# 30stomercury/whisper-char-alignment

Measured on AMD Instinct MI355X. Metric: utterances/sec (whisper-medium, 10s audio, char align) at 1/2/4/8 MI355X, higher is better.
Workload: dtype f16x2 (hi + lo operand pairs on the f16 MFMA pipe: fp32-equivalent operands, fp32 accumulate)

## Files before the change

whisper-char-alignment_amd/csrc/gemm.hip:

```cpp
#include <atomic>

#include "gemm_epilogue.h"
#include <cstdlib>
#include "kernels.h"
#include "wca_common.h"

namespace wca {

namespace {

constexpr int BM = 128, BN = 128, BK = 64;
constexpr int TILE_ELEMS = 128 * 64;

struct RowPtrs {
  const half_t* p[4];
};

__device__ __forceinline__ half8 ldfrag(const half_t* tile, int r, int c) {
  return *reinterpret_cast<const half8*>(tile + r * 64 + ((c ^ swz128(r)) << 3));
}

template <int OUT_MODE, bool GELU, int MT>
__device__ __forceinline__ void epilogue(const GemmArgs& a, f32x4 (&acc)[MT][4], int mbase, int nb, int fr) {
  float bv[16];
#pragma unroll
  for (int j = 0; j < 16; ++j) bv[j] = (a.bias != nullptr && nb + j < a.N) ? a.bias[nb + j] : 0.f;
  const bool full_n = (nb + 16 <= a.N);

#pragma unroll
  for (int mt = 0; mt < MT; ++mt) {
    const int m = mbase + mt * 16 + fr;
    if (m >= a.M) continue;
    float v[16];
#pragma unroll
    for (int nt = 0; nt < 4; ++nt)
#pragma unroll
      for (int r = 0; r < 4; ++r) v[nt * 4 + r] = acc[mt][nt][r] + bv[nt * 4 + r];
    if (OUT_MODE != 2 && a.addend != nullptr) {
      const float* ap = a.addend + (long)m * a.ld_addend + nb;
#pragma unroll
      for (int j = 0; j < 16; ++j)
        if (nb + j < a.N) v[j] += ap[j];
    }
    if (GELU) {
#pragma unroll
      for (int j = 0; j < 16; j += 2) {
        if (OUT_MODE == 4) {
          const f32x2 g = gelu_erfc2(f32x2{v[j], v[j + 1]});
          v[j] = g[0];
          v[j + 1] = g[1];
        } else {
          v[j] = gelu_erf(v[j]);
          v[j + 1] = gelu_erf(v[j + 1]);
        }
      }
    }
    if (a.pos != nullptr) {
      const float* pp = a.pos + (long)(m % a.pos_period) * a.N + nb;
#pragma unroll
      for (int j = 0; j < 16; ++j)
        if (nb + j < a.N) v[j] += pp[j];
    }
    long coff;
    if (a.c_rows_per_batch > 0) {
      const int b = m / a.c_rows_per_batch;
      const int t = m - b * a.c_rows_per_batch;
      coff = (long)b * a.c_batch_stride + (long)t * a.ldc;
    } else {
      coff = (long)m * a.ldc;
    }
    if (OUT_MODE == 0 || OUT_MODE == 4) {
      half_t* cp = reinterpret_cast<half_t*>(a.C) + coff + nb;
      if (full_n && ((reinterpret_cast<uintptr_t>(cp) & 15) == 0)) {
        half8 h0, h1, l0, l1;
        if (OUT_MODE == 4) {
#pragma unroll
          for (int j = 0; j < 8; j += 2) {
            const Half2Pair p0 = split_pair2(v[j], v[j + 1]), p1 = split_pair2(v[8 + j], v[8 + j + 1]);
            h0[j] = p0.hi[0];
            h0[j + 1] = p0.hi[1];
            l0[j] = p0.lo[0];
            l0[j + 1] = p0.lo[1];
            h1[j] = p1.hi[0];
            h1[j + 1] = p1.hi[1];
            l1[j] = p1.lo[0];
            l1[j + 1] = p1.lo[1];
          }
        } else {
#pragma unroll
          for (int j = 0; j < 8; ++j) {
            h0[j] = (half_t)v[j];
            h1[j] = (half_t)v[8 + j];
          }
        }
        reinterpret_cast<half8*>(cp)[0] = h0;
        reinterpret_cast<half8*>(cp)[1] = h1;
        if (OUT_MODE == 4) {
          reinterpret_cast<half8*>(cp + a.c_lo)[0] = l0;
          reinterpret_cast<half8*>(cp + a.c_lo)[1] = l1;
        }
      } else {
#pragma unroll
        for (int j = 0; j < 16; ++j)
          if (nb + j < a.N) {
            if (OUT_MODE == 4) {
              const HalfPair pr = split_pair(v[j]);
              cp[j] = pr.hi;
              cp[a.c_lo + j] = pr.lo;
            } else {
              cp[j] = (half_t)v[j];
            }
          }
      }
    } else {
      float* cp = reinterpret_cast<float*>(a.C) + coff + nb;
      if (full_n && ((reinterpret_cast<uintptr_t>(cp) & 15) == 0)) {
        f32x4* c4 = reinterpret_cast<f32x4*>(cp);
#pragma unroll
        for (int q = 0; q < 4; ++q) {
          f32x4 o = f32x4{v[q * 4 + 0], v[q * 4 + 1], v[q * 4 + 2], v[q * 4 + 3]};
          if (OUT_MODE == 2) o += c4[q];
          c4[q] = o;
        }
      } else {
#pragma unroll
        for (int j = 0; j < 16; ++j)
          if (nb + j < a.N) cp[j] = (OUT_MODE == 2) ? cp[j] + v[j] : v[j];
      }
    }
  }
}

template <int OUT_MODE, bool GELU, int SITE>
__global__ __launch_bounds__(256, 2) void gemm_f16_kernel(GemmArgs a) {
  extern __shared__ __attribute__((aligned(16))) char smem[];
  half_t* lds = reinterpret_cast<half_t*>(smem);
  const int tid = threadIdx.x;
  const int lane = tid & 63;
  const int wave = __builtin_amdgcn_readfirstlane(tid >> 6);
  const int wm = wave >> 1, wn = wave & 1;

  const int ntn = (a.N + BN - 1) / BN;
  const int ntm = (a.M + BM - 1) / BM;
  const int nwg = ntm * ntn;
  const int id = xcd_remap(blockIdx.x, nwg);
  const int tm = id / ntn, tn = id - tm * ntn;
  const int m0 = tm * BM, n0 = tn * BN;

  const half_t* asrc[4];
  const half_t* wsrc[4];
#pragma unroll
  for (int i = 0; i < 4; ++i) {
    const int r = (wave * 4 + i) * 8 + (lane >> 3);
    const int c = (lane & 7) ^ swz128(r);
    int gm = m0 + r;
    gm = gm < a.M ? gm : a.M - 1;
    long aoff;
    if (a.a_rows_per_batch > 0) {
      const int b = gm / a.a_rows_per_batch;
      const int t = gm - b * a.a_rows_per_batch;
      aoff = (long)b * a.a_batch_stride + (long)t * a.lda;
    } else {
      aoff = (long)gm * a.lda;
    }
    const int kbeg = (int)blockIdx.y * (a.K / (int)gridDim.y);
    asrc[i] = a.A + aoff + c * 8 + kbeg;
    int gn = n0 + r;
    gn = gn < a.N ? gn : a.N - 1;
    wsrc[i] = a.W + (long)gn * a.ldw + c * 8 + kbeg;
  }

  auto stage = [&](int buf, int k0) {
    half_t* At = lds + buf * (2 * TILE_ELEMS);
    half_t* Wt = At + TILE_ELEMS;
#pragma unroll
    for (int i = 0; i < 4; ++i) {
      const int rbase = (wave * 4 + i) * 8;
      glds16(asrc[i] + k0, At + rbase * 64);
      glds16(wsrc[i] + k0, Wt + rbase * 64);
    }
  };

  f32x4 acc[4][4];
#pragma unroll
  for (int i = 0; i < 4; ++i)
#pragma unroll
    for (int j = 0; j < 4; ++j) acc[i][j] = f32x4{0.f, 0.f, 0.f, 0.f};

  const int fr = lane & 15;
  const int fg = lane >> 4;
  int xrow[4], wrow[4];
#pragma unroll
  for (int t = 0; t < 4; ++t) {
    xrow[t] = wm * 64 + t * 16 + fr;
    wrow[t] = wn * 64 + (fr >> 2) * 16 + t * 4 + (fr & 3);
  }

  const int nk = a.K / BK / (int)gridDim.y;
  stage(0, 0);
  wait_vm0();
  __syncthreads();
  int cur = 0;
  for (int kt = 0; kt < nk; ++kt) {
    if (kt + 1 < nk) stage(cur ^ 1, (kt + 1) * BK);
    const half_t* At = lds + cur * (2 * TILE_ELEMS);
    const half_t* Wt = At + TILE_ELEMS;
#pragma unroll
    for (int ks = 0; ks < 2; ++ks) {
      half8 xf[4], wf[4];
#pragma unroll
      for (int t = 0; t < 4; ++t) {
        xf[t] = ldfrag(At, xrow[t], ks * 4 + fg);
        wf[t] = ldfrag(Wt, wrow[t], ks * 4 + fg);
      }
#pragma unroll
      for (int mt = 0; mt < 4; ++mt)
#pragma unroll
        for (int nt = 0; nt < 4; ++nt)
          acc[mt][nt] = __builtin_amdgcn_mfma_f32_16x16x32_f16(wf[nt], xf[mt], acc[mt][nt], 0, 0, 0);
    }
    wait_vm0();
    __syncthreads();
    cur ^= 1;
  }

  if (OUT_MODE == 2 && gridDim.y > 1) {
    GemmArgs p = a;
    p.C = a.sk_part + (long)blockIdx.y * a.M * a.N;
    p.ldc = a.N;
    p.c_rows_per_batch = 0;
    p.bias = nullptr;
    p.pos = nullptr;
    epilogue<1, false, 4>(p, acc, m0 + wm * 64, n0 + wn * 64 + fg * 16, fr);
    return;
  }
  epilogue<OUT_MODE, GELU, 4>(a, acc, m0 + wm * 64, n0 + wn * 64 + fg * 16, fr);
}

__global__ __launch_bounds__(256) void splitk_reduce_kernel(const float* __restrict__ part, int S, int M, int N, const float* __restrict__ bias,
                                                            float* __restrict__ x, int ldc) {
  const long i4 = (long)blockIdx.x * blockDim.x + threadIdx.x;
  const int n4 = N >> 2;
  if (i4 >= (long)M * n4) return;
  const int m = (int)(i4 / n4), n = (int)(i4 - (long)m * n4) * 4;
  f32x4 v = *reinterpret_cast<const f32x4*>(part + (long)m * N + n);
  for (int s = 1; s < S; ++s) v += *reinterpret_cast<const f32x4*>(part + ((long)s * M + m) * N + n);
  if (bias != nullptr) v += *reinterpret_cast<const f32x4*>(bias + n);
  f32x4* xp = reinterpret_cast<f32x4*>(x + (long)m * ldc + n);
  *xp = *xp + v;
}


template <int OUT_MODE, bool GELU, int SITE>
__global__ __launch_bounds__(512) void gemm256_f16_kernel(GemmArgs a) {
  extern __shared__ __attribute__((aligned(16))) char smem[];
  half_t* lds = reinterpret_cast<half_t*>(smem);
  constexpr int TILE256 = 256 * 64;
  const int tid = threadIdx.x;
  const int lane = tid & 63;
  const int wave = __builtin_amdgcn_readfirstlane(tid >> 6);
  const int wr = wave >> 2, wc = wave & 3;

  const int ntn = (a.N + 255) / 256;
  const int ntm = (a.M + 255) / 256;
  const int nwg = ntm * ntn;
  const int id = xcd_remap(blockIdx.x, nwg);
  const int tm = id / ntn, tn = id - tm * ntn;
  const int m0 = tm * 256, n0 = tn * 256;

  const half_t* asrc[4];
  const half_t* wsrc[4];
#pragma unroll
  for (int i = 0; i < 4; ++i) {
    const int r = (wave * 4 + i) * 8 + (lane >> 3);
    const int c = (lane & 7) ^ swz128(r);
    int gm = m0 + r;
    gm = gm < a.M ? gm : a.M - 1;
    long aoff;
    if (a.a_rows_per_batch > 0) {
      const int b = gm / a.a_rows_per_batch;
      const int t = gm - b * a.a_rows_per_batch;
      aoff = (long)b * a.a_batch_stride + (long)t * a.lda;
    } else {
      aoff = (long)gm * a.lda;
    }
    asrc[i] = a.A + aoff + c * 8;
    int gn = n0 + r;
    gn = gn < a.N ? gn : a.N - 1;
    wsrc[i] = a.W + (long)gn * a.ldw + c * 8;
  }

  auto stage = [&](int buf, int k0) {
    half_t* At = lds + buf * (2 * TILE256);
    half_t* Wt = At + TILE256;
#pragma unroll
    for (int i = 0; i < 4; ++i) {
      const int rbase = (wave * 4 + i) * 8;
      glds16(asrc[i] + k0, At + rbase * 64);
      glds16(wsrc[i] + k0, Wt + rbase * 64);
    }
  };

  f32x4 acc[8][4];
#pragma unroll
  for (int i = 0; i < 8; ++i)
#pragma unroll
    for (int j = 0; j < 4; ++j) acc[i][j] = f32x4{0.f, 0.f, 0.f, 0.f};

  const int fr = lane & 15, fg = lane >> 4;
  int xrow[8], wrow[4];
#pragma unroll
  for (int t = 0; t < 8; ++t) xrow[t] = wr * 128 + t * 16 + fr;
#pragma unroll
  for (int t = 0; t < 4; ++t) wrow[t] = wc * 64 + (fr >> 2) * 16 + t * 4 + (fr & 3);

  const int nk = a.K / BK;
  stage(0, 0);
  if (nk > 1) stage(1, BK);
  for (int kt = 0; kt < nk; ++kt) {
    const int cur = kt & 1;
    const half_t* At = lds + cur * (2 * TILE256);
    const half_t* Wt = At + TILE256;
    if (kt + 1 < nk) {
      asm volatile("s_waitcnt vmcnt(8)" ::: "memory");
    } else {
      asm volatile("s_waitcnt vmcnt(0)" ::: "memory");
    }
    __builtin_amdgcn_s_barrier();
    asm volatile("" ::: "memory");

    half8 wf[2][4], xf[2][4];
#pragma unroll
    for (int ks = 0; ks < 2; ++ks)
#pragma unroll
      for (int t = 0; t < 4; ++t) {
        wf[ks][t] = ldfrag(Wt, wrow[t], ks * 4 + fg);
        xf[ks][t] = ldfrag(At, xrow[t], ks * 4 + fg);
      }
    __builtin_amdgcn_s_setprio(1);
#pragma unroll
    for (int ks = 0; ks < 2; ++ks)
#pragma unroll
      for (int mt = 0; mt < 4; ++mt)
#pragma unroll
        for (int nt = 0; nt < 4; ++nt)
          acc[mt][nt] = __builtin_amdgcn_mfma_f32_16x16x32_f16(wf[ks][nt], xf[ks][mt], acc[mt][nt], 0, 0, 0);
    __builtin_amdgcn_s_setprio(0);

    half8 xg[2][4];
#pragma unroll
    for (int ks = 0; ks < 2; ++ks)
#pragma unroll
      for (int t = 0; t < 4; ++t) xg[ks][t] = ldfrag(At, xrow[4 + t], ks * 4 + fg);
    asm volatile("s_waitcnt lgkmcnt(0)" ::: "memory");
    __builtin_amdgcn_s_barrier();
    asm volatile("" ::: "memory");
    if (kt + 2 < nk) stage(cur, (kt + 2) * BK);
    __builtin_amdgcn_s_setprio(1);
#pragma unroll
    for (int ks = 0; ks < 2; ++ks)
#pragma unroll
      for (int mt = 0; mt < 4; ++mt)
#pragma unroll
        for (int nt = 0; nt < 4; ++nt)
          acc[4 + mt][nt] = __builtin_amdgcn_mfma_f32_16x16x32_f16(wf[ks][nt], xg[ks][mt], acc[4 + mt][nt], 0, 0, 0);
    __builtin_amdgcn_s_setprio(0);
  }

  epilogue<OUT_MODE, GELU, 8>(a, acc, m0 + wr * 128, n0 + wc * 64 + fg * 16, fr);
}

template <int V>
struct GemmIntC {
  static constexpr int value = V;
};

template <int OUT_MODE, bool GELU, int SITE, int SPLITW_MODE = 0>
__global__ __launch_bounds__(512) void gemm256p_f16_kernel(GemmArgs a) {
  constexpr bool SPLITW = SPLITW_MODE != 0;
  constexpr bool RING3 = SPLITW_MODE == 2;
  extern __shared__ __attribute__((aligned(16))) char smem[];
  half_t* lds = reinterpret_cast<half_t*>(smem);
  constexpr int TILE256 = 256 * 64;
  float* bias_lds = reinterpret_cast<float*>(smem + 4 * TILE256 * sizeof(half_t));
  float* gamma_lds = bias_lds + 512;
  float* beta_lds = gamma_lds + 512;
  float* ln_lds = beta_lds + 512;
  const int tid = threadIdx.x;
  const int lane = tid & 63;
  const int wave = __builtin_amdgcn_readfirstlane(tid >> 6);
  const int wr = wave >> 2, wc = wave & 3;

  const int ntn = (a.N + 255) / 256;
  const int ntm = (a.M + 255) / 256;
  const int nwg = ntm * ntn;
  const int G = gridDim.x;

  const __amdgpu_buffer_rsrc_t ra = __builtin_amdgcn_make_buffer_rsrc(const_cast<half_t*>(a.A), 0, (int)a.a_bytes, 0x00020000);
  const __amdgpu_buffer_rsrc_t rw = __builtin_amdgcn_make_buffer_rsrc(const_cast<half_t*>(a.W), 0, (int)a.w_bytes, 0x00020000);
  const __amdgpu_buffer_rsrc_t rb = __builtin_amdgcn_make_buffer_rsrc(const_cast<float*>(a.bias), 0, a.bias != nullptr ? a.N * 4 : 0, 0x00020000);
  const __amdgpu_buffer_rsrc_t rg = __builtin_amdgcn_make_buffer_rsrc(const_cast<float*>(a.ln_gamma), 0, OUT_MODE == 3 ? a.N * 4 : 0, 0x00020000);
  const __amdgpu_buffer_rsrc_t rbeta = __builtin_amdgcn_make_buffer_rsrc(const_cast<float*>(a.ln_beta), 0, OUT_MODE == 3 ? a.N * 4 : 0, 0x00020000);
  const int l8 = lane >> 3;
  const int rho = wave * 8 + l8;
  const int c0 = (lane & 7) ^ ((rho >> 1) & 7);
  const int nt_r = rho >> 4, i_r = rho & 15;
  const int wsrc_row = (OUT_MODE == 0 || OUT_MODE == 3 || OUT_MODE == 4) ? ((nt_r >> 1) * 32 + (i_r >> 2) * 8 + (nt_r & 1) * 4 + (i_r & 3)) : rho;
  const unsigned va = (unsigned)(rho * a.lda + c0 * 8) * 2u;
  const unsigned vw = (unsigned)(wsrc_row * a.ldw + c0 * 8) * 2u;
  const unsigned sa64 = 64u * a.lda * 2u, sw64 = 64u * a.ldw * 2u;

  auto a_slot = [&](int buf) -> half_t* { return RING3 ? lds + buf * TILE256 : lds + buf * (2 * TILE256); };
  auto w_slot = [&](int bufw) -> half_t* { return RING3 ? lds + 3 * TILE256 : lds + bufw * (2 * TILE256) + TILE256; };
  auto stage_one = [&](int buf, int bufw, unsigned ta, unsigned tw, int g) {
    half_t* At = a_slot(buf);
    half_t* Wt = w_slot(bufw);
    const int i = g >> 1;
    unsigned so = ((g & 1) == 0) ? ta + i * sa64 : tw + i * sw64;
    asm volatile("" : "+s"(so));
    if ((g & 1) == 0)
      __builtin_amdgcn_raw_ptr_buffer_load_lds(ra, (WCA_LDS void*)(At + (i * 64 + wave * 8) * 64), 16, (int)(va + so), 0, 0, 0);
    else
      __builtin_amdgcn_raw_ptr_buffer_load_lds(rw, (WCA_LDS void*)(Wt + (i * 64 + wave * 8) * 64), 16, (int)(vw + so), 0, 0, 0);
  };

  auto stage_bias = [&](int par, int ncol0) {
    if (wave < 4) {
      __builtin_amdgcn_raw_ptr_buffer_load_lds(rb, (WCA_LDS void*)(bias_lds + par * 256 + wave * 64), 4, (ncol0 + wave * 64 + lane) * 4, 0, 0, 0);
      if (OUT_MODE == 3) {
        __builtin_amdgcn_raw_ptr_buffer_load_lds(rg, (WCA_LDS void*)(gamma_lds + par * 256 + wave * 64), 4, (ncol0 + wave * 64 + lane) * 4, 0, 0, 0);
        __builtin_amdgcn_raw_ptr_buffer_load_lds(rbeta, (WCA_LDS void*)(beta_lds + par * 256 + wave * 64), 4, (ncol0 + wave * 64 + lane) * 4, 0, 0, 0);
      }
    }
  };
  constexpr int RING3_A_REQS_IN_FLIGHT = 4;
  static_assert(RING3_A_REQS_IN_FLIGHT * 64 == 256, "one request per 64-row block of the 256-row A tile");

  const int fr = lane & 15, fg = lane >> 4;
  const int pos0 = fg ^ ((fr >> 1) & 7);
  const int xb0 = (wr * 128 + fr) * 64 + pos0 * 8, xb1 = (wr * 128 + fr) * 64 + (pos0 ^ 4) * 8;
  const int wb0 = (wc * 64 + fr) * 64 + pos0 * 8, wb1 = (wc * 64 + fr) * 64 + (pos0 ^ 4) * 8;

#define WCA_LOAD_HALF(AT, WT, XB, WB, WF, XF)                                                      \
  do {                                                                                             \
    _Pragma("unroll") for (int t = 0; t < 4; ++t) WF[t] = *reinterpret_cast<const half8*>((WT) + (WB) + t * 1024); \
    _Pragma("unroll") for (int t = 0; t < 8; ++t) XF[t] = *reinterpret_cast<const half8*>((AT) + (XB) + t * 1024); \
  } while (0)

  const int nk = SPLITW ? 2 * (a.K / BK) : a.K / BK;
  auto a_koff = [&](int s_) -> unsigned {
    return SPLITW ? (unsigned)(((s_ & 1) * (int)a.a_lo + (s_ >> 1) * BK) * 2) : (unsigned)(s_ * (BK * 2));
  };
  auto w_koff = [&](int s_) -> unsigned {
    return SPLITW ? (unsigned)((s_ >> 1) * (BK * 2)) : (unsigned)(s_ * (BK * 2));
  };
  int v = blockIdx.x;
  int id = xcd_remap(v, nwg);
  const int SM = a.supertile > 0 ? a.supertile : 1;
  auto tile_of = [&](int t, int& tm, int& tn) {
    const int per = SM * ntn;
    const int st = t / per, r = t - st * per;
    const int rows = (ntm - st * SM) < SM ? (ntm - st * SM) : SM;
    tn = r / rows;
    tm = st * SM + (r - tn * rows);
  };
  const int spx = G >> 3;
  const int PR = spx / ntn;
  const int lab = blockIdx.x & 7, slot = blockIdx.x >> 3;
  const int pq = ntm >> 3, prm = ntm & 7;
  const int lab_panels = pq + (lab < prm ? 1 : 0), lab_base = lab * pq + (lab < prm ? lab : prm);
  auto tile_of_round = [&](int round, int& tm, int& tn) -> bool {
    tn = slot / PR;
    const int pi = round * PR + (slot - tn * PR);
    tm = lab_base + pi;
    return tn < ntn && pi < lab_panels;
  };
  int tm_, tn_;
  int round = 0;
  if (OUT_MODE == 3) {
    if (!tile_of_round(0, tm_, tn_)) return;
  } else {
    tile_of(id, tm_, tn_);
  }
  int m0 = tm_ * 256, n0 = tn_ * 256;
  unsigned ta = (unsigned)m0 * a.lda * 2u, tw = (unsigned)n0 * a.ldw * 2u;

  f32x4 acc[8][4];
#pragma unroll
  for (int i = 0; i < 8; ++i)
#pragma unroll
    for (int j = 0; j < 4; ++j) acc[i][j] = f32x4{0.f, 0.f, 0.f, 0.f};
  half8 w0[4], x0[8], w1[4], x1[8];
  int par = 0;
  stage_bias(0, n0);
#pragma unroll
  for (int g = 0; g < 8; ++g) stage_one(0, 0, ta, tw, g);
  if (nk > 1) {
#pragma unroll
    for (int g = 0; g < 8; ++g)
      if (!SPLITW || (g & 1) == 0) stage_one(1, 1, ta + a_koff(1), tw + w_koff(1), g);
    if (SPLITW) asm volatile("s_waitcnt vmcnt(4)" ::: "memory");
    else asm volatile("s_waitcnt vmcnt(8)" ::: "memory");
  } else {
    asm volatile("s_waitcnt vmcnt(0)" ::: "memory");
  }
  __builtin_amdgcn_s_barrier();
  asm volatile("" ::: "memory");
  WCA_LOAD_HALF(a_slot(0), w_slot(0), xb0, wb0, w0, x0);
  int ring_a = 0;

  for (;;) {
    const int vn = v + G;
    bool has_next;
    int idn = id;
    int tmn_, tnn_;
    if (OUT_MODE == 3) {
      has_next = tile_of_round(round + 1, tmn_, tnn_);
      if (!has_next) {
        tmn_ = m0 >> 8;
        tnn_ = n0 >> 8;
      }
    } else {
      has_next = vn < nwg;
      idn = has_next ? xcd_remap(vn, nwg) : id;
      tile_of(idn, tmn_, tnn_);
    }
    const int m0n = tmn_ * 256, n0n = tnn_ * 256;
    const unsigned tan = (unsigned)m0n * a.lda * 2u, twn = (unsigned)n0n * a.ldw * 2u;
    auto kstep = [&](auto par_c, const int kt) {
      constexpr int PAR = decltype(par_c)::value;
      const int cur = RING3 ? ring_a : (PAR >= 0 ? PAR : (kt & 1));
      const int nxt = RING3 ? (ring_a == 2 ? 0 : ring_a + 1) : (cur ^ 1);
      const int wslot = SPLITW ? ((kt >> 1) & 1) : cur;
      const int wslot_n = SPLITW ? (((kt + 1) >> 1) & 1) : (cur ^ 1);
      const bool W_FRESH = !SPLITW || (PAR >= 0 ? PAR == 0 : (kt & 1) == 0);
      const bool W_NEXT_FRESH = !SPLITW || (PAR >= 0 ? PAR == 1 : (kt & 1) == 1);
      const half_t* At = a_slot(cur);
      const half_t* Wt = w_slot(wslot);
      const bool in_tile2 = kt + 2 < nk;
      const bool more1 = kt + 1 < nk, more2 = in_tile2 || has_next;
      const unsigned ka = (in_tile2 ? ta + a_koff(kt + 2) : tan + a_koff(kt + 2 - nk));
      const unsigned kw = (in_tile2 ? tw + w_koff(kt + 2) : twn + w_koff(kt + 2 - nk));
      const int prv = RING3 ? (ring_a == 0 ? 2 : ring_a - 1) : 0;
#pragma unroll
      for (int g = 0; g < 8; ++g) {
        __builtin_amdgcn_s_setprio(1);
#pragma unroll
        for (int nt = 0; nt < 4; ++nt) acc[g][nt] = __builtin_amdgcn_mfma_f32_16x16x32_f16(w0[nt], x0[g], acc[g][nt], 0, 0, 0);
        __builtin_amdgcn_s_setprio(0);
        __builtin_amdgcn_sched_barrier(0);
        if (g < 2) {
          if (W_FRESH) {
            w1[2 * g] = *reinterpret_cast<const half8*>(Wt + wb1 + (2 * g) * 1024);
            w1[2 * g + 1] = *reinterpret_cast<const half8*>(Wt + wb1 + (2 * g + 1) * 1024);
          }
        } else if (g < 6) {
          x1[2 * (g - 2)] = *reinterpret_cast<const half8*>(At + xb1 + (2 * (g - 2)) * 1024);
          x1[2 * (g - 2) + 1] = *reinterpret_cast<const half8*>(At + xb1 + (2 * (g - 2) + 1) * 1024);
        }
        if (RING3 && (g & 1) == 0 && (g >> 1) < RING3_A_REQS_IN_FLIGHT && more2) stage_one(prv, 0, ka, kw, g);
        __builtin_amdgcn_sched_barrier(0);
      }
      if (RING3 && more2) asm volatile("s_waitcnt vmcnt(%0) lgkmcnt(0)" ::"i"(RING3_A_REQS_IN_FLIGHT) : "memory");
      else asm volatile("s_waitcnt vmcnt(0) lgkmcnt(0)" ::: "memory");
      __builtin_amdgcn_s_barrier();
      asm volatile("" ::: "memory");
      const int wslot_2 = SPLITW ? (wslot ^ 1) : cur;
      const half_t* An = a_slot(nxt);
      const half_t* Wn = w_slot(wslot_n);
#pragma unroll
      for (int g = 0; g < 8; ++g) {
        __builtin_amdgcn_s_setprio(1);
#pragma unroll
        for (int nt = 0; nt < 4; ++nt) acc[g][nt] = __builtin_amdgcn_mfma_f32_16x16x32_f16(w1[nt], x1[g], acc[g][nt], 0, 0, 0);
        __builtin_amdgcn_s_setprio(0);
        __builtin_amdgcn_sched_barrier(0);
        if (RING3) {
          if (W_FRESH && (g & 1) == 1 && more2) stage_one(cur, 0, ka, kw, g);
        } else if (more2 && (W_FRESH || (g & 1) == 0)) {
          stage_one(cur, wslot_2, ka, kw, g);
        }
        if (more1) {
          if (g < 2) {
            if (W_NEXT_FRESH) {
              w0[2 * g] = *reinterpret_cast<const half8*>(Wn + wb0 + (2 * g) * 1024);
              w0[2 * g + 1] = *reinterpret_cast<const half8*>(Wn + wb0 + (2 * g + 1) * 1024);
            }
          } else if (g < 6) {
            x0[2 * (g - 2)] = *reinterpret_cast<const half8*>(An + xb0 + (2 * (g - 2)) * 1024);
            x0[2 * (g - 2) + 1] = *reinterpret_cast<const half8*>(An + xb0 + (2 * (g - 2) + 1) * 1024);
          }
        }
        __builtin_amdgcn_sched_barrier(0);
      }
      if (RING3) ring_a = nxt;
    };
    for (int kt = 0; kt < nk; ++kt) kstep(GemmIntC<-1>{}, kt);

    {
      int fr_e = fr, fg_e = fg;
      asm volatile("" : "+v"(fr_e), "+v"(fg_e));
      typedef __attribute__((address_space(4))) GemmArgs KernArgs;
      const KernArgs* ap = (const KernArgs*)__builtin_amdgcn_kernarg_segment_ptr();
      asm volatile("" : "+s"(ap));
      if constexpr (OUT_MODE == 3)
        epilogue_ln<KernArgs>(*ap, acc, m0, m0 >> 8, n0 >> 8, ntn, wr, wc, fr_e, fg_e, bias_lds + par * 256 + wc * 64, gamma_lds + par * 256,
                              beta_lds + par * 256, ln_lds);
      else
        epilogue_wide<OUT_MODE, GELU, KernArgs>(*ap, acc, m0 + wr * 128, n0 + wc * 64, fr_e, fg_e, bias_lds + par * 256 + wc * 64);
    }
    if (!has_next) break;
    par ^= 1;
    stage_bias(par, n0n);
    v = vn;
    id = idn;
    ++round;
    m0 = m0n;
    n0 = n0n;
    ta = tan;
    tw = twn;
#pragma unroll
    for (int i = 0; i < 8; ++i)
#pragma unroll
      for (int j = 0; j < 4; ++j) acc[i][j] = f32x4{0.f, 0.f, 0.f, 0.f};
    WCA_LOAD_HALF(a_slot(RING3 ? ring_a : 0), w_slot(0), xb0, wb0, w0, x0);
  }
#undef WCA_LOAD_HALF
}


template <int OUT_MODE, bool GELU>
__global__ __launch_bounds__(256) void gemm_skinny_f16_kernel(GemmArgs a) {
  __shared__ float red[4][4][4][64];
  const int tid = threadIdx.x;
  const int lane = tid & 63;
  const int wave = __builtin_amdgcn_readfirstlane(tid >> 6);
  const int fr = lane & 15, fg = lane >> 4;
  const int n0 = blockIdx.x * 16;
  const int kq = a.K >> 2;
  const int kbeg = wave * kq;
  int nrow = n0 + fr;
  nrow = nrow < a.N ? nrow : a.N - 1;
  const half_t* wp = a.W + (long)nrow * a.ldw + kbeg + fg * 8;
  const half_t* xp[4];
#pragma unroll
  for (int mt = 0; mt < 4; ++mt) {
    int m = mt * 16 + fr;
    m = m < a.M ? m : a.M - 1;
    xp[mt] = a.A + (long)m * a.lda + kbeg + fg * 8;
  }
  f32x4 acc[4];
#pragma unroll
  for (int mt = 0; mt < 4; ++mt) acc[mt] = f32x4{0.f, 0.f, 0.f, 0.f};
  half8 wf[2][4], xf[2][4][4];
  auto load_chunk = [&](int buf, int k) {
#pragma unroll
    for (int u = 0; u < 4; ++u) {
      wf[buf][u] = *reinterpret_cast<const half8*>(wp + k + u * 32);
#pragma unroll
      for (int mt = 0; mt < 4; ++mt) xf[buf][u][mt] = *reinterpret_cast<const half8*>(xp[mt] + k + u * 32);
    }
  };
  auto mul_chunk = [&](int buf) {
#pragma unroll
    for (int u = 0; u < 4; ++u)
#pragma unroll
      for (int mt = 0; mt < 4; ++mt) acc[mt] = __builtin_amdgcn_mfma_f32_16x16x32_f16(wf[buf][u], xf[buf][u][mt], acc[mt], 0, 0, 0);
  };
  load_chunk(0, 0);
  for (int k = 0; k < kq; k += 256) {
    if (k + 128 < kq) load_chunk(1, k + 128);
    mul_chunk(0);
    if (k + 256 < kq) load_chunk(0, k + 256);
    if (k + 128 < kq) mul_chunk(1);
  }
#pragma unroll
  for (int mt = 0; mt < 4; ++mt)
#pragma unroll
    for (int r = 0; r < 4; ++r) red[wave][mt][r][lane] = acc[mt][r];
  __syncthreads();
  const int m = wave * 16 + fr;
  float v[4];
#pragma unroll
  for (int r = 0; r < 4; ++r) v[r] = red[0][wave][r][lane] + red[1][wave][r][lane] + red[2][wave][r][lane] + red[3][wave][r][lane];
  if (m >= a.M) return;
  const int nb = n0 + 4 * fg;
#pragma unroll
  for (int r = 0; r < 4; ++r) {
    const int n = nb + r;
    if (a.bias != nullptr && n < a.N) v[r] += a.bias[n];
    if (GELU) v[r] = gelu_erf(v[r]);
  }
  long coff;
  if (a.c_rows_per_batch > 0) {
    const int b = m / a.c_rows_per_batch;
    coff = (long)b * a.c_batch_stride + (long)(m - b * a.c_rows_per_batch) * a.ldc;
  } else {
    coff = (long)m * a.ldc;
  }
  if (OUT_MODE == 0) {
    half_t* cp = reinterpret_cast<half_t*>(a.C) + coff + nb;
    if (nb + 4 <= a.N && (reinterpret_cast<uintptr_t>(cp) & 7) == 0) {
      half4 o;
#pragma unroll
      for (int r = 0; r < 4; ++r) o[r] = (half_t)v[r];
      *reinterpret_cast<half4*>(cp) = o;
    } else {
#pragma unroll
      for (int r = 0; r < 4; ++r)
        if (nb + r < a.N) cp[r] = (half_t)v[r];
    }
  } else {
    float* cp = reinterpret_cast<float*>(a.C) + coff + nb;
#pragma unroll
    for (int r = 0; r < 4; ++r)
      if (nb + r < a.N) cp[r] = (OUT_MODE == 2) ? cp[r] + v[r] : v[r];
  }
}

}

bool gemm_ln_supported(int M, int N, int K, int n_cu) {
  if (N % 256 != 0 || N > 2048 || K % 128 != 0 || M < 1) return false;
  const long tiles = (long)((M + 255) / 256) * (N / 256);
  if (tiles < 192) return false;
  return (n_cu >> 3) >= N / 256;
}

bool gemm_splitw_supported(int M, int N, int K, int lda, int out_mode) {
  if (M < 1 || N < 1 || K < 128 || (K % 128) != 0) return false;
  if (out_mode != 0 && out_mode != 1 && out_mode != 2 && out_mode != 4) return false;
  const long tiles256 = (long)((M + 255) / 256) * ((N + 255) / 256);
  if (tiles256 < 192) return false;
  const size_t a_need = ((size_t)(M - 1) * lda + 2 * (size_t)K) * sizeof(half_t), w_need = ((size_t)(N - 1) * K + K) * sizeof(half_t);
  return a_need < 0x7fffffffull && w_need < 0x7fffffffull;
}

hipError_t launch_gemm(const GemmArgs& a_in, hipStream_t s) {
  GemmArgs a = a_in;
  if (a.M <= 0 || a.N <= 0) return hipSuccess;
  if (a.K <= 0 || (a.K % BK) != 0) return hipErrorInvalidValue;
  if ((a.lda % 8) != 0 || (a.ldw % 8) != 0) return hipErrorInvalidValue;
  if (a.out_mode == 4 && (a.c_lo <= 0 || (a.c_lo & 7))) return hipErrorInvalidValue;
  if (a.addend != nullptr && (a.out_mode == 2 || a.out_mode == 3 || a.a_lo > 0)) return hipErrorInvalidValue;
  if ((a.force_tile == 64 || a.force_tile == 0) && a.M <= 64 && (a.K % 512) == 0 && a.a_rows_per_batch == 0 && a.pos == nullptr && a.addend == nullptr && a.out_mode != 4 && a.a_lo <= 0) {
    const dim3 sgrid((unsigned)((a.N + 15) / 16)), sblock(256);
#define WCA_LAUNCH_SK(OM, G) hipLaunchKernelGGL((gemm_skinny_f16_kernel<OM, G>), sgrid, sblock, 0, s, a)
    if (a.out_mode == 0) {
      if (a.gelu) WCA_LAUNCH_SK(0, true); else WCA_LAUNCH_SK(0, false);
    } else if (a.out_mode == 1) {
      if (a.gelu) WCA_LAUNCH_SK(1, true); else WCA_LAUNCH_SK(1, false);
    } else if (a.out_mode == 2 && !a.gelu) {
      WCA_LAUNCH_SK(2, false);
    } else {
      return hipErrorInvalidValue;
    }
#undef WCA_LAUNCH_SK
    return hipGetLastError();
  }
  if (a.force_tile == 64) return hipErrorInvalidValue;
  const long tiles256 = (long)((a.M + 255) / 256) * ((a.N + 255) / 256);
  const bool splitw = a.a_lo > 0;
  if (splitw && (a.force_tile == 64 || a.force_tile == 128 || a.force_tile == 256 || a.a_rows_per_batch != 0 ||
                 !gemm_splitw_supported(a.M, a.N, a.K, a.lda, a.out_mode) || (a.a_lo & 7) != 0))
    return hipErrorInvalidValue;
  const size_t a_need = ((size_t)(a.M - 1) * a.lda + (splitw ? (size_t)a.a_lo : 0) + a.K) * sizeof(half_t), w_need = ((size_t)(a.N - 1) * a.ldw + a.K) * sizeof(half_t);
  const bool can_buf = a.a_rows_per_batch == 0 && a_need < 0x7fffffffull && w_need < 0x7fffffffull;
  if (a.a_bytes == 0) a.a_bytes = (unsigned)a_need;
  if (a.w_bytes == 0) a.w_bytes = (unsigned)w_need;
  int dev = 0;
  {
    hipError_t e = hipGetDevice(&dev);
    if (e != hipSuccess) return e;
  }
  static std::atomic<int> n_cu_cache[32] = {};
  int n_cu = n_cu_cache[dev & 31].load(std::memory_order_relaxed);
  if (n_cu == 0) {
    hipError_t e = hipDeviceGetAttribute(&n_cu, hipDeviceAttributeMultiprocessorCount, dev);
    if (e != hipSuccess) return e;
    n_cu_cache[dev & 31].store(n_cu, std::memory_order_relaxed);
  }
  if (a.cu_limit > 0 && a.cu_limit < n_cu) n_cu = a.cu_limit;
  const int ring = splitw ? (debug_switch(DBG_GEMM_RING) == 1 ? 1 : 2) : 0;
  const bool want_big = (a.force_tile == 256 || a.force_tile == 257 || a.force_tile == 258) || (a.force_tile == 0 && tiles256 >= 192);
  const bool pipelined = want_big && can_buf && a.force_tile != 256 && a.addend == nullptr;
  const bool big = want_big;
  dim3 grid, block;
  size_t shmem;
  int splitk = 1;
  if (big) {
    grid = dim3((unsigned)tiles256);
    block = dim3(512);
    shmem = 2 * 2 * 256 * 64 * sizeof(half_t);
    if (pipelined) {
      shmem += 2 * 256 * sizeof(float);
      const int nk = (splitw ? 2 : 1) * (a.K / BK);
      if (a.force_tile != 258 && nk >= 2 && (nk & 1) == 0 && tiles256 > n_cu) grid = dim3((unsigned)n_cu);
      if (a.supertile <= 0) a.supertile = ((splitw ? 2 : 1) * a.K <= 2048 && (a.N + 255) / 256 <= 32) ? 8 : 1;
    }
  } else {
    const int ntn = (a.N + BN - 1) / BN, ntm = (a.M + BM - 1) / BM;
    grid = dim3(ntn * ntm);
    block = dim3(256);
    shmem = 2 * 2 * TILE_ELEMS * sizeof(half_t);
    splitk = 1;
    if (a.out_mode == 2 && !a.gelu && a.sk_part != nullptr && a.pos == nullptr && a.c_rows_per_batch == 0 && (a.N % 4) == 0 && (a.ldc % 4) == 0 &&
        ntn * ntm <= n_cu / 2 && a.K >= 2048) {
      for (int sk = 4; sk >= 2; --sk)
        if (a.K % (sk * BK) == 0 && (size_t)sk * a.M * a.N * sizeof(float) <= a.sk_bytes) {
          splitk = sk;
          break;
        }
    }
    grid.y = (unsigned)splitk;
  }
#define WCA_LAUNCH_K(...)                                                                         \
  do {                                                                                            \
    static std::atomic<unsigned> attr_mask{0};                                                    \
    if (!(attr_mask.load(std::memory_order_acquire) & (1u << (dev & 31)))) {                      \
      hipError_t e = hipFuncSetAttribute(reinterpret_cast<const void*>(__VA_ARGS__),              \
                                         hipFuncAttributeMaxDynamicSharedMemorySize, (int)shmem); \
      if (e != hipSuccess) return e;                                                              \
      attr_mask.fetch_or(1u << (dev & 31), std::memory_order_release);                            \
    }                                                                                             \
    hipLaunchKernelGGL((__VA_ARGS__), grid, block, shmem, s, a);                                  \
  } while (0)
#define WCA_LAUNCH_S(OM, G, S)                            \
  do {                                                    \
    if (pipelined && splitw && ring == 1) { if ((S) == 4) WCA_LAUNCH_K(gemm256p_f16_kernel<OM, G, 4, 1>); else WCA_LAUNCH_K(gemm256p_f16_kernel<OM, G, 1, 1>); } \
    else if (pipelined && splitw) { if ((S) == 4) WCA_LAUNCH_K(gemm256p_f16_kernel<OM, G, 4, 2>); else if ((S) == 3) WCA_LAUNCH_K(gemm256p_f16_kernel<OM, G, 3, 2>); else if ((S) == 2) WCA_LAUNCH_K(gemm256p_f16_kernel<OM, G, 2, 2>); else WCA_LAUNCH_K(gemm256p_f16_kernel<OM, G, 1, 2>); } \
    else if (pipelined) WCA_LAUNCH_K(gemm256p_f16_kernel<OM, G, S>); \
    else if (big) WCA_LAUNCH_K(gemm256_f16_kernel<OM, G, S>);  \
    else WCA_LAUNCH_K(gemm_f16_kernel<OM, G, S>);         \
  } while (0)
#define WCA_LAUNCH(OM, G)                     \
  do {                                        \
    switch (a.site) {                         \
      case 1: WCA_LAUNCH_S(OM, G, 1); break;  \
      case 2: WCA_LAUNCH_S(OM, G, 2); break;  \
      case 3: WCA_LAUNCH_S(OM, G, 3); break;  \
      case 4: WCA_LAUNCH_S(OM, G, 4); break;  \
      default: WCA_LAUNCH_S(OM, G, 0); break; \
    }                                         \
  } while (0)
  if (a.out_mode == 3) {
    if (!gemm_ln_supported(a.M, a.N, a.K, n_cu) || a.gelu || !pipelined || a.force_tile == 258 || a.pos != nullptr || a.c_rows_per_batch != 0 || !a.ln_gamma ||
        !a.ln_beta || !a.ln_out || !a.ln_stats || !a.ln_cnt || (a.ldc & 3) || (a.ln_ld & 7))
      return hipErrorInvalidValue;
    const size_t cnt_bytes = (((size_t)((a.M + 255) / 256) * sizeof(unsigned)) + 15) / 16 * 16;
    hipError_t e = hipMemsetAsync(a.ln_cnt, 0, cnt_bytes, s);
    if (e != hipSuccess) return e;
    shmem += (2 * 512 + 2560) * sizeof(float);
    grid = dim3((unsigned)(n_cu & ~7));
    switch (a.site) {
      case 4: WCA_LAUNCH_K(gemm256p_f16_kernel<3, false, 4>); break;
      default: WCA_LAUNCH_K(gemm256p_f16_kernel<3, false, 1>); break;
    }
  } else if (a.out_mode == 0) {
    if (a.gelu) WCA_LAUNCH(0, true); else WCA_LAUNCH(0, false);
  } else if (a.out_mode == 1) {
    if (a.gelu) WCA_LAUNCH(1, true); else WCA_LAUNCH(1, false);
  } else if (a.out_mode == 2) {
    if (a.gelu) return hipErrorInvalidValue;
    WCA_LAUNCH(2, false);
  } else if (a.out_mode == 4) {
    if (a.gelu) WCA_LAUNCH(4, true); else WCA_LAUNCH(4, false);
  } else {
    return hipErrorInvalidValue;
  }
#undef WCA_LAUNCH
#undef WCA_LAUNCH_S
#undef WCA_LAUNCH_K
  {
    hipError_t e = hipGetLastError();
    if (e != hipSuccess) return e;
  }
  if (splitk > 1) {
    const long n4 = (long)a.M * (a.N / 4);
    hipLaunchKernelGGL(splitk_reduce_kernel, dim3((unsigned)((n4 + 255) / 256)), dim3(256), 0, s, a.sk_part, splitk, a.M, a.N, a.bias,
                       reinterpret_cast<float*>(a.C), a.ldc);
  }
  return hipGetLastError();
}

}
```

Measured before the change: 343.5.

## Deepen GEMM K-loop prefetch to two tiles ahead with partial vmcnt waits

Restructures the GEMM main loop so two K tiles are in flight. Each iteration waits only for the current tile's global loads (vmcnt(8)), reads all fragments into registers, then barriers. It then issues the load for tile kt+2 into the freed LDS buffer before running the MFMAs. The goal is to hide global-load latency behind compute instead of draining all loads at the end of every iteration. In exchange it uses more fragment registers, and it depends on stage() issuing exactly 8 VMEM ops per thread for the hardcoded vmcnt to be correct.

Measured after the change: 342.8 (median of 2 runs). Within noise of the previous version (-0.2%).

```diff
diff --git a/whisper-char-alignment_amd/csrc/gemm.hip b/whisper-char-alignment_amd/csrc/gemm.hip
--- a/whisper-char-alignment_amd/csrc/gemm.hip
+++ b/whisper-char-alignment_amd/csrc/gemm.hip
@@ -198,30 +198,37 @@
 
   const int nk = a.K / BK / (int)gridDim.y;
   stage(0, 0);
-  wait_vm0();
-  __syncthreads();
-  int cur = 0;
+  if (nk > 1) stage(1, BK);
   for (int kt = 0; kt < nk; ++kt) {
-    if (kt + 1 < nk) stage(cur ^ 1, (kt + 1) * BK);
+    const int cur = kt & 1;
     const half_t* At = lds + cur * (2 * TILE_ELEMS);
     const half_t* Wt = At + TILE_ELEMS;
-#pragma unroll
-    for (int ks = 0; ks < 2; ++ks) {
-      half8 xf[4], wf[4];
+    if (kt + 1 < nk) {
+      asm volatile("s_waitcnt vmcnt(8)" ::: "memory");
+    } else {
+      asm volatile("s_waitcnt vmcnt(0)" ::: "memory");
+    }
+    __builtin_amdgcn_s_barrier();
+    asm volatile("" ::: "memory");
+    half8 xf[2][4], wf[2][4];
+#pragma unroll
+    for (int ks = 0; ks < 2; ++ks)
 #pragma unroll
       for (int t = 0; t < 4; ++t) {
-        xf[t] = ldfrag(At, xrow[t], ks * 4 + fg);
-        wf[t] = ldfrag(Wt, wrow[t], ks * 4 + fg);
+        xf[ks][t] = ldfrag(At, xrow[t], ks * 4 + fg);
+        wf[ks][t] = ldfrag(Wt, wrow[t], ks * 4 + fg);
       }
+    asm volatile("s_waitcnt lgkmcnt(0)" ::: "memory");
+    __builtin_amdgcn_s_barrier();
+    asm volatile("" ::: "memory");
+    if (kt + 2 < nk) stage(cur, (kt + 2) * BK);
+#pragma unroll
+    for (int ks = 0; ks < 2; ++ks)
 #pragma unroll
       for (int mt = 0; mt < 4; ++mt)
 #pragma unroll
         for (int nt = 0; nt < 4; ++nt)
-          acc[mt][nt] = __builtin_amdgcn_mfma_f32_16x16x32_f16(wf[nt], xf[mt], acc[mt][nt], 0, 0, 0);
-    }
-    wait_vm0();
-    __syncthreads();
-    cur ^= 1;
+          acc[mt][nt] = __builtin_amdgcn_mfma_f32_16x16x32_f16(wf[ks][nt], xf[ks][mt], acc[mt][nt], 0, 0, 0);
   }
 
   if (OUT_MODE == 2 && gridDim.y > 1) {
```
